# samson6460/tf2_YOLO

Hardware: AMD Instinct MI355X
Metric: images/sec training YOLOv3 416x416 bs=32/GPU (higher is better)
Workload: dtype f32-storage/fp16x2-mfma

## Files before the change

### include/yolo_hip.h

```cpp
#ifndef YOLO_HIP_H_
#define YOLO_HIP_H_

#include <stddef.h>
#include <stdint.h>

#ifdef __cplusplus
extern "C" {
#endif

typedef enum yolo_status {
  YOLO_OK = 0,
  YOLO_ERR_INVALID_ARG = -1,
  YOLO_ERR_LAUNCH = -2,
  YOLO_ERR_WORKSPACE = -3
} yolo_status;

enum { YOLO_ACT_LINEAR = 0, YOLO_ACT_LEAKY = 1, YOLO_ACT_MISH = 2 };
enum { YOLO_HEAD_V3 = 3, YOLO_HEAD_V2 = 2, YOLO_HEAD_V1 = 1, YOLO_HEAD_V4 = 4 };
enum { YOLO_NMS_HARD = 1, YOLO_NMS_SOFT = 2, YOLO_NMS_DIOU = 3 };

const char* yolo_last_error(void);
int yolo_abi_version(void);
int yolo_device_available(void);
int yolo_mfma_probe(const void* operands_f16, float* sink, int workgroups, int iters, double* flops_host, void* stream);

enum { YOLO_OPT_CONV_WIN = 0, YOLO_OPT_STAMPS = 1, YOLO_OPT_CONV_SK = 2, YOLO_OPT_CONV_PATCH = 5, YOLO_OPT_WGRAD_WIN = 6,
       YOLO_OPT_NMS_WALK = 7 ,
       YOLO_OPT_AB = 8  };
int yolo_set_option(int key, int value);
const char* yolo_last_conv_kernel(int* launches_host);
size_t yolo_conv_workspace_bytes(void);
int yolo_set_conv_workspace(void* p, size_t bytes, void* stream);
int yolo_set_debug_buffer(void* p, size_t bytes);

typedef struct yolo_conv_desc {
  int N, H, W, Cin;
  int Cout, kh, kw;
  int Ho, Wo;
  int sh, sw;
  int pad_t, pad_l;
} yolo_conv_desc;

#define YOLO_BN_STAT_SLOTS 64
#define YOLO_BN_RED_SLOTS 512
#define YOLO_SPLIT_BATCH_UNITS 4

int yolo_conv2d_fwd(const yolo_conv_desc* d, const float* x, const float* w,
                    const float* bias, float* y, double* stats, void* stream);
int yolo_conv2d_fwd_absmax(const yolo_conv_desc* d, const float* x, const float* w, const float* bias,
                           float* y, double* stats, unsigned* absmax, void* stream);

int yolo_conv2d_dgrad(const yolo_conv_desc* d, const float* dy, const float* wT,
                      float* dx, int accumulate, void* stream);

int yolo_conv2d_wgrad(const yolo_conv_desc* d, const float* x, const float* dy,
                      float* dw, float* dbias, void* stream);

int yolo_conv2d_wgrad_bias(const float* dy, long long P, int Cout, float* dbias, void* stream);

int yolo_filter_transpose(const float* w, float* wT, int Cout, int taps, int Cin, void* stream);

size_t yolo_planes_bytes(long long rows, int C);
// ... 303 lines not shown
```

### tf2_yolo_amd/_lib.py

```python
import ctypes
import os
from ctypes import (POINTER, Structure, c_char_p, c_double, c_float, c_int, c_longlong,
                    c_size_t, c_void_p)

from . import tape as _tape

_HERE = os.path.dirname(os.path.abspath(__file__))
LIB_PATH = os.path.join(_HERE, "libyolo_hip.so")

ACT_LINEAR, ACT_LEAKY, ACT_MISH = 0, 1, 2
PREC_F32, PREC_F16 = 0, 1
_PRECISIONS = {"fp32": PREC_F32, "fp16": PREC_F16}


def precision_enum(precision):
    try:
        return _PRECISIONS[precision]
    except (KeyError, TypeError):
        raise ValueError(f"precision must be 'fp32' or 'fp16', got {precision!r}") from None
NMS_HARD, NMS_SOFT, NMS_DIOU = 1, 2, 3


class YoloHipError(RuntimeError):
    pass


class ConvDesc(Structure):
    _fields_ = [(n, c_int) for n in
                ("N", "H", "W", "Cin", "Cout", "kh", "kw", "Ho", "Wo", "sh", "sw", "pad_t", "pad_l")]


class LossCfg(Structure):
    _fields_ = [("version", c_int), ("N", c_int), ("gh", c_int), ("gw", c_int), ("A", c_int),
                ("C", c_int), ("anchors", c_float * 32), ("use_anchors", c_int),
                ("binary_weight", c_float), ("loss_weight", c_float * 4),
                ("ignore_thresh", c_float), ("use_focal_loss", c_int), ("focal_gamma", c_float),
                ("use_scale", c_int), ("wh_reg_weight", c_float), ("truth_thresh", c_float),
                ("label_smooth", c_float)]


_P = c_void_p
_LL = c_longlong
SIGNATURES = {
    "yolo_last_error": (c_char_p, []),
    "yolo_abi_version": (c_int, []),
    "yolo_device_available": (c_int, []),
    "yolo_set_option": (c_int, [c_int, c_int]),
    "yolo_last_conv_kernel": (c_char_p, [POINTER(c_int)]),
    "yolo_mfma_probe": (c_int, [_P, _P, c_int, c_int, POINTER(c_double), _P]),
    "yolo_set_debug_buffer": (c_int, [_P, c_size_t]),
    "yolo_encode_labels": (c_int, [_P, _P, _P, c_int, c_double, c_double, c_int, c_int, c_int, _P, _P, _P]),
    "yolo_down2xlabel": (c_int, [_P, c_int, c_int, c_int, c_int, _P, _P, _P]),
    "yolo_conv_workspace_bytes": (c_size_t, []),
    "yolo_set_conv_workspace": (c_int, [_P, c_size_t, _P]),
    "yolo_conv2d_fwd": (c_int, [POINTER(ConvDesc), _P, _P, _P, _P, _P, _P]),
    "yolo_conv2d_dgrad": (c_int, [POINTER(ConvDesc), _P, _P, _P, c_int, _P]),
    "yolo_conv2d_wgrad": (c_int, [POINTER(ConvDesc), _P, _P, _P, _P, _P]),
    "yolo_conv2d_wgrad_bias": (c_int, [_P, _LL, c_int, _P, _P]),
    "yolo_filter_transpose": (c_int, [_P, _P, c_int, c_int, c_int, _P]),
    "yolo_planes_bytes": (c_size_t, [_LL, c_int]),
    "yolo_split_planes": (c_int, [_P, _LL, c_int, _P, _P]),
    "yolo_split_planes_padded": (c_int, [_P, _LL, c_int, c_int, _P, _P]),
    "yolo_split_planes_batch": (c_int, [_P, c_int, _LL, _P]),
    "yolo_filter_transpose_batch": (c_int, [_P, c_int, _LL, _P]),
    "yolo_conv2d_fwd_planes": (c_int, [POINTER(ConvDesc), _P, _P, _P, _P, _P, _P, _P]),
    "yolo_stem_bwd_scratch_bytes": (c_size_t, []),
    "yolo_stem_bn_bwd_wgrad": (c_int, [POINTER(ConvDesc), _P, _P, _P, _P, _P, _P, _P, c_int, _P, _P, _P, _P, _P, c_size_t, _P]),
    "yolo_conv2d_fwd_planes_epi": (c_int, [POINTER(ConvDesc), _P, _P, _P, c_int, _P, _P, _P, _P, _P, _P]),
    "yolo_split_planes_absmax": (c_int, [_P, _LL, c_int, _P, _P, _P, _P, _P]),
    "yolo_conv_pred_bound": (c_int, [_P, c_int, c_int, _P, _P, _P, _P, _P]),
    "yolo_conv2d_fwd_infer_unit": (c_int, [POINTER(ConvDesc), _P, _P, _P, c_int, _P, _P, _P, _P, _P, _P, _P, c_int, _P, c_int,
                                           _P, _P, _P, POINTER(c_int), _P]),
    "yolo_fold_bound": (c_int, [_P, c_int, _P, _P]),
    "yolo_absmax_words": (c_int, [_P, _LL, _P, POINTER(c_int), _P]),
    "yolo_stem_filter_prep": (c_int, [_P, _P, _P, _P]),
    "yolo_stem_fwd_infer_unit": (c_int, [POINTER(ConvDesc), _P, _P, c_int, _P, _P, _P, _P, c_int, _P, _P, _P, POINTER(c_int), _P]),
    "yolo_split_planes_concat": (c_int, [POINTER(c_void_p), POINTER(c_int), POINTER(c_void_p), c_int, _LL, _P, _P, _P, _P]),
    "yolo_split_planes_concat_ex": (c_int, [POINTER(c_void_p), POINTER(c_int), POINTER(c_void_p), POINTER(c_int), POINTER(c_int),
                                            c_int, c_int, c_int, _LL, _P, _P, _P, _P]),
    "yolo_conv2d_fwd_head_unit": (c_int, [POINTER(ConvDesc), _P, _P, _P, c_int, c_int, c_int, _P, _P, _P, _P]),
# ... 78 lines not shown
    "yolo_nms_workspace_bytes": (c_size_t, [c_int, c_int]),
    "yolo_cal_iou": (c_int, [_P, _P, _P, _P, c_int, c_int, c_int, POINTER(c_longlong), POINTER(c_longlong),
                             POINTER(c_longlong), c_double, c_double, _P]),
    "yolo_match_detections": (c_int, [_P, c_int, _P, c_int, c_int, c_double, _P, _P, _P, _P, _P, _P]),
    "yolo_rank_desc": (c_int, [_P, _P, c_int, _P, _P]),
    "yolo_pr_curve_workspace_bytes": (c_size_t, [c_int, c_int]),
    "yolo_pr_curve": (c_int, [_P, _P, _P, c_int, c_int, c_int, _P, c_size_t, _P, _P, _P]),
    "yolo_match_batch_workspace_bytes": (c_size_t, [c_int, c_int, c_int]),
    "yolo_match_batch": (c_int, [_P, c_int, _P, _P, c_int, _P, c_int, c_int, c_double, _P, _P, _P, _P, _P, _P, _P, c_size_t, _P]),
    "yolo_rank_desc_images": (c_int, [_P, _P, c_int, _P, c_int, _P, _P]),
    "yolo_pr_curves_workspace_bytes": (c_size_t, [c_int, c_int, _LL]),
    "yolo_pr_curves": (c_int, [_P, _P, _P, _P, c_int, _P, c_int, _LL, c_int, _P, c_size_t, _P, _P, _P, _P]),
    "yolo_nms": (c_int, [_P, c_int, c_int, c_int, c_double, c_double, c_double, _P, _P, c_size_t, _P]),
    "yolo_nms_select": (c_int, [_P, c_int, c_int, c_int, c_double, c_double, c_double, _P, _P, _P, _P, c_size_t, _P]),
    "yolo_decode_batch_workspace_bytes": (c_size_t, [c_int, POINTER(c_int), POINTER(c_int), POINTER(c_int), c_int, c_int]),
    "yolo_decode_batch_count": (c_int, [POINTER(c_void_p), POINTER(c_int), c_int, c_int, POINTER(c_int), POINTER(c_int),
                                        POINTER(c_int), c_int, c_int, POINTER(c_double), _P, _P, c_size_t, _P]),
    "yolo_decode_batch_write": (c_int, [POINTER(c_void_p), POINTER(c_int), c_int, c_int, POINTER(c_int), POINTER(c_int),
                                        POINTER(c_int), c_int, c_int, POINTER(c_double), _P, c_int, _P, c_size_t, _P]),
    "yolo_nms_batch_workspace_bytes": (c_size_t, [c_int, c_int, c_int]),
    "yolo_nms_batch_prepare": (c_int, [_P, c_int, _P, c_int, c_int, _P, _P, c_size_t, _P]),
    "yolo_nms_batch_select": (c_int, [_P, c_int, c_int, c_int, c_int, c_double, c_double, c_double, _P, _LL, _P, _P, _P, _P,
                                      c_size_t, _P]),
    "yolo_image_prepare": (c_int, [_P, _LL, _P, c_int, c_int, c_int, c_float, c_float, _P, _P]),
}

_lib = None

_QUERIES = {"yolo_last_error", "yolo_last_conv_kernel", "yolo_abi_version", "yolo_bnred_slots_cap", "yolo_device_available", "yolo_conv_workspace_bytes", "yolo_planes_bytes",
            "yolo_stem_bwd_scratch_bytes", "yolo_loss_workspace_bytes", "yolo_decode_workspace_bytes",
            "yolo_nms_workspace_bytes", "yolo_pr_curve_workspace_bytes", "yolo_wgrad_workspace_bytes", "yolo_adam_lr_t",
            "yolo_grad_sqnorm_workspace_bytes", "yolo_decode_batch_workspace_bytes", "yolo_nms_batch_workspace_bytes",
            "yolo_match_batch_workspace_bytes", "yolo_pr_curves_workspace_bytes",
            "yolo_set_option", "yolo_set_debug_buffer", "yolo_set_conv_workspace", "yolo_set_wgrad_workspace"}


class _Recorded:
    __slots__ = ("f", "name")

    def __init__(self, f, name):
        self.f, self.name = f, name

    def __call__(self, *a):
        rc = self.f(*a)
        if _tape.ACTIVE is not None:
            _tape.ACTIVE.c(self.f, a, self.name)
        return rc


class _Lib:

    def __init__(self, cdll):
        self._cdll = cdll

    def __getattr__(self, name):
        f = getattr(self._cdll, name)
        if name not in _QUERIES and name in SIGNATURES:
            f = _Recorded(f, name)
        setattr(self, name, f)
        return f


def load():
    global _lib
    if _lib is not None:
        return _lib
    if not os.path.exists(LIB_PATH):
# ... 24 lines not shown
```

### tf2_yolo_amd/csrc/conv_args.hpp

```cpp
#pragma once
#include "common.hpp"

namespace yolo {

constexpr int MAX_TAPS = 49;

struct Tap {
  int oy, ox, woff;
};

struct ClassGeom {
  long long M;
  int Hg, Wg, ooy, oox, tap0, ntaps;
};

struct GatherConvArgs {
  const float* src;
  const float* wgt;
  const float* bias;
  float* dst;
  double* stats;
  unsigned* absmax;
  long long M;
  int N, Hs, Ws, Cs;
// ... 68 lines not shown
  long long M;
  int N, Hs, Ws, Cs;
  int Hg, Wg;
  int sy, sx;
  int Cout, ldw;
  int ntaps;
  int kw, pad_t, pad_l;
  int tiles_co, tiles_j;
  int nblocks;
  long long chunk;
  unsigned src_bytes, dy_bytes;
  int zero_blk_src, zero_blk_dy;
  float* slabs;
  int splits;
};

int launch_gather_split(GatherConvArgs& a, hipStream_t st);
bool gather_split_supported(const GatherConvArgs& a);
long long planes_bytes(long long rows, int C);
int launch_split_planes(const float* x, long long rows, int C, void* planes, hipStream_t st);
int launch_split_planes_absmax(const float* x, long long rows, int C, const unsigned* absmax, const float* extra_bound, int extra_n,
                               void* planes, float* out_bound, hipStream_t st);
int launch_split_planes_concat(const float* const* xs, const int* Cs, const float* const* bounds, int nsrc, long long rows,
                               void* planes, float* dst32, float* out_bound, hipStream_t st,
                               const int* bound_words = nullptr, const int* upsample = nullptr, int H = 0, int W = 0);
int launch_split_planes_padded(const float* x, long long rows, int Csrc, int C, void* planes, hipStream_t st);
int launch_split_planes_batch(const void* jobs, int njobs, long long total_blocks, hipStream_t st);
int launch_filter_transpose_batch(const void* jobs, int njobs, long long total_blocks, hipStream_t st);
int launch_gather_planes(GatherConvArgs& a, hipStream_t st);
bool conv_small_supported(const GatherConvArgs& a);
bool conv_small_head_supported(const GatherConvArgs& a);
int launch_conv_small(GatherConvArgs& a, hipStream_t st, int* nwg);
bool gather_planes_supported(const GatherConvArgs& a);
int conv_split_parts(const GatherConvArgs& a, long long nb, int bm, int min_cb, int idle_div);
int launch_split_reduce(GatherConvArgs& a, int bm, hipStream_t st);
float* conv_split_slabs();
int launch_conv_win(GatherConvArgs& a, int variant, hipStream_t st);
bool conv_win_supported(const GatherConvArgs& a);
enum { OPT_CONV_WIN = 0, OPT_STAMPS = 1, OPT_CONV_SK = 2, OPT_DBG = 3, OPT_TILE_ORDER = 4, OPT_CONV_PATCH = 5, OPT_WGRAD_WIN = 6, OPT_NMS_WALK = 7, OPT_EXP = 8, OPT_COUNT = 16 };
int set_conv_workspace(void* p, size_t bytes, hipStream_t st);
extern void* g_dbg_buf;
extern size_t g_dbg_bytes;
extern int g_opt[OPT_COUNT];
void init_options();
void note_conv_launch(const char* family, int a = 0, int b = 0, int c = 0, int d = 0);
int launch_wgrad_planes(WgradArgs& a, hipStream_t st);
bool wgrad_planes_supported(const WgradArgs& a);
int launch_wgrad_win(WgradArgs& a, hipStream_t st);
bool wgrad_win_supported(const WgradArgs& a);
constexpr size_t WGRAD_WS_COLSUM_BYTES = 1 << 20;
void* wgrad_workspace(size_t* bytes);
bool stem_fwd_supported(const yolo_conv_desc* d);
struct StemEpiArgs {
  const float* scale;
  const float* shift;
  int act;
  void* planes;
  const float* pred;
  const unsigned* in_words;
  int in_n;
  unsigned* out_words;
};
bool stem_infer_supported(const yolo_conv_desc* d);
int launch_stem_filter_prep(const float* w, const float* bias, float* wt, hipStream_t st);
int launch_absmax_words(const float* x, long long n, unsigned* words, int* n_words, hipStream_t st);
int launch_stem_infer(const yolo_conv_desc* d, const float* x, const float* wt, float* y, const StemEpiArgs& e, int* out_n,
                      hipStream_t st);
size_t stem_bwd_scratch_bytes();
int launch_stem_bn_bwd_wgrad(const yolo_conv_desc* d, const float* y, const float* dout, const float* img, const float* scale,
                             const float* shift, const float* smean, const float* sinv, int act, const double* redsum,
                             float* dgamma, float* dbeta, float* dw, float* scratch, size_t scratch_bytes, hipStream_t st);
int launch_stem_fwd(const yolo_conv_desc* d, const float* x, const float* w, const float* bias, float* y, double* stats,
// ... 6 lines not shown
```

### tf2_yolo_amd/csrc/conv_planes.hip

```cpp
#include "planes_epilogue.hpp"
#include <algorithm>
#include <cstdlib>
#include <type_traits>

namespace yolo {

__global__ __launch_bounds__(256) void planes_amax_kernel(const float* __restrict__ x, long long n4,
                                                         unsigned* __restrict__ header) {
  float m = 0.f;
  for (long long i = (long long)blockIdx.x * 256 + threadIdx.x; i < n4; i += (long long)gridDim.x * 256) {
    const f32x4 v = reinterpret_cast<const f32x4*>(x)[i];
    m = fmaxf(fmaxf(m, fmaxf(fabsf(v[0]), fabsf(v[1]))), fmaxf(fabsf(v[2]), fabsf(v[3])));
  }
#pragma unroll
  for (int o = 32; o > 0; o >>= 1) m = fmaxf(m, __shfl_xor(m, o, 64));
  __shared__ float wmax[4];
  if ((threadIdx.x & 63) == 0) wmax[threadIdx.x >> 6] = m;
  __syncthreads();
  if (threadIdx.x == 0) {
    m = fmaxf(fmaxf(wmax[0], wmax[1]), fmaxf(wmax[2], wmax[3]));
    if (__builtin_bit_cast(unsigned, m) > *reinterpret_cast<volatile unsigned*>(header))
      atomicMax(header, __builtin_bit_cast(unsigned, m));
  }
}
// ... 198 lines not shown
                                                                 long long rows_padded) {
  unsigned* header = reinterpret_cast<unsigned*>(out + planes_body_bytes(rows, C));
  const float sc = planes_scale_from_bound(header[0]);
  const int G = C >> 3;
  const long long t = (long long)blockIdx.x * 256 + threadIdx.x;
  if (t == 0) {
    reinterpret_cast<float*>(header)[1] = sc;
    reinterpret_cast<float*>(header)[2] = 1.f / sc;
  }
  if (t >= rows_padded * G) return;
  const long long row = t / G;
  const int g = (int)(t - row * G);
  f32x4 v0 = {0.f, 0.f, 0.f, 0.f}, v1 = {0.f, 0.f, 0.f, 0.f};
  if (row < rows) {
    const float* p = x + row * Csrc;
#pragma unroll
    for (int j = 0; j < 4; ++j) {
      if (g * 8 + j < Csrc) v0[j] = p[g * 8 + j];
      if (g * 8 + 4 + j < Csrc) v1[j] = p[g * 8 + 4 + j];
    }
  }
  const Planes8 s = split8(v0, v1, sc);
  unsigned char* o = out + planes_unit_offset(row, g, C);
  *reinterpret_cast<u32x4*>(o) = s.h;
  *reinterpret_cast<u32x4*>(o + 512) = s.l;
}

constexpr int PF_KO_MASK = 31;
constexpr int PF_SPLIT = 32;
constexpr int PF_MULTI = 64;
constexpr int PF_DEEP1 = 128;
constexpr int PF_DEEP2 = 256;
constexpr int PF_BNRED = 512;
template <int BM, int BN, int WGM, int WGN, int FORM = 0, int PASSES = 3>
__global__ __launch_bounds__(64 * WGM * WGN, (WGM * WGN >= 4 ? 2 : 1)) void gather_conv_planes_kernel(const GatherConvArgs a) {
  static_assert(planes_passes_ok(PASSES), "1 or 3 MFMA passes");
  static_assert(PASSES == 3 || (FORM & (PF_MULTI | PF_BNRED)) == 0, "one pass: forward inference forms only");
  constexpr int NPL = planes_frag_planes<PASSES>;
  constexpr int NW = WGM * WGN;
  constexpr int TM = BM / WGM / 32;
  constexpr int TN = BN / WGN / 32;
  constexpr int RBA = BM / 32, RBB = BN / 32;
  constexpr int LPW = (RBA + RBB + NW - 1) / NW;
  static_assert(LPW <= 4, "loader layout: slot s = wave + i*NW loads A block s, or B block (s - RBA) % RBB");
  constexpr int ND = PL_PLANES * LPW;
  constexpr int STAGE_BYTES = (RBA + RBB) * PL_PLANES * 1024;
  constexpr int NBUF = 3 + ((FORM >> 7) & 3);

  extern __shared__ __attribute__((aligned(16))) unsigned char smem[];
  const unsigned lds_base = (unsigned)(size_t)smem;

  const int tid = threadIdx.x;
  const int lane = tid & 63;
  const int wave = __builtin_amdgcn_readfirstlane(tid >> 6);
  const int wm = wave / WGN, wn = wave % WGN;

  constexpr bool SPLIT = (FORM & PF_SPLIT) != 0;
  const int SP = SPLIT ? a.split_parts : 1;
  const int part = SPLIT ? (int)blockIdx.x / a.nblocks : 0;
  const int tile = xcd_remap(SPLIT ? (int)blockIdx.x - part * a.nblocks : (int)blockIdx.x, a.nblocks);
  constexpr bool MULTI = (FORM & PF_MULTI) != 0;
  constexpr bool BNRED = (FORM & PF_BNRED) != 0;
  const int tile_n = tile % a.tiles_n;
  const int cls = MULTI ? (tile / a.tiles_n) % a.ncls : 0;
  const int tile_m = MULTI ? tile / (a.tiles_n * a.ncls) : tile / a.tiles_n;
  const long long m0 = (long long)tile_m * BM;
  const int n0 = tile_n * BN;
  const EpiGeom G = MULTI ? EpiGeom{a.cls[cls].M, a.cls[cls].Hg, a.cls[cls].Wg, a.cls[cls].ooy, a.cls[cls].oox, 0, 0, 0,
                                    tile_m * a.ncls + cls + 1}
                          : epi_geom_of(a);
  const int tap0 = MULTI ? a.cls[cls].tap0 : 0;
  const int ntaps = MULTI ? a.cls[cls].ntaps : a.ntaps;
  if (MULTI && m0 >= G.M) {
    if (a.bwd_y != nullptr)
      for (int c = tid; c < BN; c += 64 * NW)
        if (n0 + c < a.Cout) {
          a.bwd_part[((long long)(G.slot1 - 1) * 2 + 0) * a.Cout + n0 + c] = 0.f;
          a.bwd_part[((long long)(G.slot1 - 1) * 2 + 1) * a.Cout + n0 + c] = 0.f;
        }
    return;
  }
  const int HgWg = G.Hg * G.Wg;

  const int r = lane & 31, hf = lane >> 5;
  const unsigned blkstrideA = (unsigned)((a.Cs >> 4) * PL_RECORD);
  const unsigned blkstrideB = (unsigned)((a.ldw >> 4) * PL_RECORD);
  const i32x4 rsrcA = planes_rsrc(a.src, a.src_bytes), rsrcB = planes_rsrc(a.wgt, a.wgt_bytes);
  const int cpt_all = a.Cs >> 4;
  const int cb_lo = (part * cpt_all) / SP;
  const int cpt = ((part + 1) * cpt_all) / SP;
  const int nk = ntaps * (cpt - cb_lo);

  bool isA[LPW];
  int nimg[LPW], ys0[LPW], xs0[LPW];
  unsigned rowbaseB[LPW], lds_mine[LPW], ld_voff[LPW], ld_soff[LPW];
#pragma unroll
  for (int i = 0; i < LPW; ++i) {
    const int slot = wave + i * NW;
    isA[i] = slot < RBA;
    const int rb = isA[i] ? slot : (slot - RBA) % RBB;
    nimg[i] = 0; ys0[i] = -(1 << 28); xs0[i] = 0; rowbaseB[i] = 0;
    if (isA[i]) {
      const long long m = m0 + rb * 32 + r;
      if (m < G.M) {
        nimg[i] = (int)(m / HgWg);
        const int rem = (int)(m - (long long)nimg[i] * HgWg);
        const int y = rem / G.Wg;
        ys0[i] = y * a.sy;
        xs0[i] = (rem - y * G.Wg) * a.sx;
      }
    } else {
      const int co = n0 + rb * 32 + r;
      const unsigned blk = co < a.Cout ? (unsigned)(co >> 4) : (unsigned)a.zero_blk_wgt;
      rowbaseB[i] = blk * blkstrideB + (co < a.Cout ? (co & 15) * 16 : 0) + hf * 256;
    }
    lds_mine[i] = lds_base + ((isA[i] ? 0 : RBA) + rb) * PL_PLANES * 1024;
    ld_voff[i] = 0; ld_soff[i] = 0;
  }

  int ld_tap = 0, ld_kk = 0, ld_cb = cb_lo;
  auto loader_tap = [&]() {
#pragma unroll
    for (int i = 0; i < LPW; ++i) {
      if (ld_cb >= cpt) {
        ld_voff[i] = isA[i] ? (unsigned)a.zero_blk_src * blkstrideA : (unsigned)a.zero_blk_wgt * blkstrideB;
        ld_soff[i] = 0;
      } else if (isA[i]) {
        const int ys = ys0[i] + a.taps[tap0 + ld_tap].oy, xs = xs0[i] + a.taps[tap0 + ld_tap].ox;
        const bool ok = ((unsigned)ys < (unsigned)a.Hs) && ((unsigned)xs < (unsigned)a.Ws);
        const int pix = (nimg[i] * a.Hs + ys) * a.Ws + xs;
        ld_voff[i] = (ok ? ((unsigned)pix >> 4) : (unsigned)a.zero_blk_src) * blkstrideA + (ok ? (pix & 15) * 16 : 0) + hf * 256;
        ld_soff[i] = (unsigned)ld_cb * PL_RECORD;
      } else {
        ld_voff[i] = rowbaseB[i];
        ld_soff[i] = (unsigned)((a.taps[tap0 + ld_tap].woff >> 4) + ld_cb) * PL_RECORD;
      }
    }
// ... 78 lines not shown
  loader_tap();
#pragma unroll
  for (int b = 0; b < NBUF; ++b) issue_stage(b);
  asm volatile("s_waitcnt vmcnt(%0)" ::"n"((NBUF - 1) * ND) : "memory");
  __builtin_amdgcn_s_barrier();
  read_frags(0, S0{});

  auto step = [&](int rbuf, int wbuf, auto CUR, auto NXT) {
    asm volatile("s_waitcnt vmcnt(%0)" ::"n"((NBUF - 2) * ND) : "memory");
    asm volatile("s_waitcnt lgkmcnt(0)" ::: "memory");
    if constexpr (!(FORM & 4)) __builtin_amdgcn_s_barrier();
    if constexpr (!(FORM & 2)) read_frags(rbuf, NXT);
    __builtin_amdgcn_sched_barrier(0);
    mfma_stage(CUR, wbuf);
  };
  {
    int rbuf = 1, wbuf = 0;
    int kt = 0;
    for (; kt + 1 < nk; kt += 2) {
      step(rbuf, wbuf, S0{}, S1{});
      rbuf = (rbuf + 1 == NBUF) ? 0 : rbuf + 1;
      wbuf = (wbuf + 1 == NBUF) ? 0 : wbuf + 1;
      step(rbuf, wbuf, S1{}, S0{});
      rbuf = (rbuf + 1 == NBUF) ? 0 : rbuf + 1;
      wbuf = (wbuf + 1 == NBUF) ? 0 : wbuf + 1;
    }
    if (kt < nk) step(rbuf, wbuf, S0{}, S1{});
  }
  asm volatile("s_waitcnt vmcnt(0)" ::: "memory");
  __syncthreads();

  if constexpr (SPLIT)
    store_split_slab<TM, TN>(a, acc, BM * BN * 4, tile * SP + part, wave, lane);
  else if constexpr (MULTI)
    planes_epilogue<BM, BN, WGM, WGN, NBUF * STAGE_BYTES, 0, NoStamp, false, BNRED>(a, acc, smem, m0, n0, tile_m, wm, wn, lane, tid, NoStamp(), &G);
  else
    planes_epilogue<BM, BN, WGM, WGN, NBUF * STAGE_BYTES, (FORM & PF_KO_MASK), NoStamp, false, BNRED>(a, acc, smem, m0, n0, tile_m, wm, wn, lane, tid);
}

template <int BM, int BN, int WGM, int WGN, int FORM = 0>
static int launch_planes(GatherConvArgs& a, hipStream_t st) {
  const long long tiles_m = (a.M + BM - 1) / BM;
  a.tiles_n = (a.Cout + BN - 1) / BN;
  const long long nb = tiles_m * a.tiles_n;
  if (nb <= 0 || nb > 0x7fffffffLL) {
    set_error("conv(planes): bad grid %lld", nb);
    return YOLO_ERR_INVALID_ARG;
  }
  note_conv_launch("gather_conv_planes_kernel<%d,%d,%d,%d>", BM, BN, WGM, WGN);
  constexpr size_t lds = (3 + ((FORM >> 7) & 3)) * (BM / 32 + BN / 32) * PL_PLANES * 1024;
  const dim3 block(64 * WGM * WGN);
  if constexpr (FORM == 0) {
    if (a.ncls > 1) {
      long long tm = 0;
      for (int c = 0; c < a.ncls; ++c) tm = std::max(tm, (a.cls[c].M + BM - 1) / BM);
      const long long nbm = tm * a.ncls * a.tiles_n;
      if (nbm <= 0 || nbm > 0x7fffffffLL) {
        set_error("conv(planes): bad grid %lld", nbm);
        return YOLO_ERR_INVALID_ARG;
      }
      a.nblocks = (int)nbm;
      a.split_parts = 1;
      a.bwd_nslots = (int)(tm * a.ncls);
      YOLO_BNRED_CHECK(a)
      if (a.bwd_y == nullptr)
        return launch_lds<gather_conv_planes_kernel<BM, BN, WGM, WGN, PF_MULTI>, lds>(dim3((unsigned)nbm), block, st, a,
                                                                                      "gather_conv_planes_kernel(classes)");
      return launch_lds<gather_conv_planes_kernel<BM, BN, WGM, WGN, PF_MULTI | PF_BNRED>, lds>(
          dim3((unsigned)nbm), block, st, a, "gather_conv_planes_kernel(classes, bn reduce)");
    }
  }
  a.nblocks = (int)nb;
  a.bwd_nslots = (int)tiles_m;
  YOLO_BNRED_CHECK(a)
  constexpr auto plain = &gather_conv_planes_kernel<BM, BN, WGM, WGN, FORM>;
  constexpr bool HAS_ONE_PASS = (FORM & ~(PF_DEEP1 | PF_DEEP2)) == 0;
  if (a.one_pass && (!HAS_ONE_PASS || a.stats != nullptr || a.bwd_y != nullptr || a.accumulate)) {
    set_error("conv(planes): one MFMA pass is an inference-forward form only");
    return YOLO_ERR_INVALID_ARG;
  }
  a.split_parts = 1;
  if constexpr (BM == 128 && BN == 128 && WGM == 2 && WGN == 2 && FORM == 0) {
    const int min_cb = a.ntaps >= 8 ? 1 : (8 + a.ntaps - 1) / a.ntaps;
    a.split_parts = conv_split_parts(a, nb, BM, min_cb, 4);
    if (a.split_parts > 1) {
      a.sk_slabs = conv_split_slabs();
      const int rc = a.one_pass ? launch_lds<gather_conv_planes_kernel<BM, BN, WGM, WGN, PF_SPLIT, 1>, lds>(
                                      dim3((unsigned)(nb * a.split_parts)), block, st, a, "gather_conv_planes_kernel(split, one pass)")
                                : launch_lds<gather_conv_planes_kernel<BM, BN, WGM, WGN, PF_SPLIT>, lds>(
                                      dim3((unsigned)(nb * a.split_parts)), block, st, a, "gather_conv_planes_kernel(split)");
      if (rc) return rc;
      return launch_split_reduce(a, BM, st);
    }
  }
  if constexpr ((FORM & ~(PF_DEEP1 | PF_DEEP2)) == 0) {
    if (a.bwd_y != nullptr)
      return launch_lds<gather_conv_planes_kernel<BM, BN, WGM, WGN, FORM | PF_BNRED>, lds>(dim3((unsigned)nb), block, st, a,
                                                                                          "gather_conv_planes_kernel(bn reduce)");
  } else if (a.bwd_y != nullptr) {
    set_error("conv(planes): this diagnostic instantiation has no fused BatchNorm-backward reduction");
    return YOLO_ERR_INVALID_ARG;
  }
  if constexpr (HAS_ONE_PASS) {
    if (a.one_pass)
      return launch_lds<gather_conv_planes_kernel<BM, BN, WGM, WGN, FORM, 1>, lds>(dim3((unsigned)nb), block, st, a,
                                                                                  "gather_conv_planes_kernel(one pass)");
  }
  return launch_lds<plain, lds>(dim3((unsigned)nb), block, st, a, "gather_conv_planes_kernel");
}

long long planes_bytes(long long rows, int C) { return planes_body_bytes(rows, C) + PL_HEADER; }

bool gather_planes_supported(const GatherConvArgs& a) { return (a.Cs % 16) == 0 && a.Cout >= 32; }

int launch_gather_planes(GatherConvArgs& a, hipStream_t st) {
  const long long rowsA = (long long)a.N * a.Hs * a.Ws;
  const long long bytesA = planes_bytes(rowsA, a.Cs), bytesB = planes_bytes(a.Cout, a.ldw);
  if (bytesA >= (1LL << 32) || bytesB >= (1LL << 32)) {
    set_error("conv(planes): operand planes exceed 4 GiB (%lld, %lld bytes)", bytesA, bytesB);
    return YOLO_ERR_INVALID_ARG;
  }
  a.src_bytes = (unsigned)bytesA;
  a.wgt_bytes = (unsigned)bytesB;
  a.zero_blk_src = (int)((rowsA + 15) / 16);
  a.zero_blk_wgt = (a.Cout + 15) / 16;
  static const int nt = env_int("YOLO_NT_STORE", 1);
  a.nt_store = nt;
  static const int vecst = env_int("YOLO_VEC_STORE", 1);
  a.vec_store = vecst;
  static const int dbg = env_int("YOLO_PLANES_DBG", 0);
  a.dbg = dbg;
  static const int kc_env = env_int("YOLO_PLANES_KC", 0);
  a.kc = kc_env > 0 ? kc_env : (a.Cs >> 4);
  if (a.kc > (a.Cs >> 4)) a.kc = a.Cs >> 4;
  init_options();
  if (g_opt[OPT_CONV_WIN] != 0 && a.ncls <= 1) {
    const int rc = launch_conv_win(a, g_opt[OPT_CONV_WIN], st);
    if (rc <= 0) return rc;
  }
  static const int deep_env = env_int("YOLO_PLANES_DEEP", -1);
  const int deep = deep_env >= 0 ? deep_env : (a.Cout <= 64 ? 1 : 2);
  if (deep && a.ntaps == 1 && a.ncls <= 1) {
    if (a.Cout <= 32) return deep == 1 ? launch_planes<128, 32, 4, 1, PF_DEEP1>(a, st) : launch_planes<128, 32, 4, 1, PF_DEEP2>(a, st);
    if (a.Cout <= 64) return deep == 1 ? launch_planes<128, 64, 4, 2, PF_DEEP1>(a, st) : launch_planes<128, 64, 4, 2, PF_DEEP2>(a, st);
  }
  if (a.Cout <= 32) return launch_planes<128, 32, 4, 1>(a, st);
  if (a.Cout <= 64) return launch_planes<128, 64, 4, 2>(a, st);
  static const int narrow_below = env_int("YOLO_PLANES_NARROW_BELOW", 0);
  if (((a.M + 127) / 128) * ((a.Cout + 127) / 128) < narrow_below) return launch_planes<128, 64, 4, 2>(a, st);
  static const int waves_env = env_int("YOLO_PLANES_WAVES", 0);
  const int waves = waves_env ? waves_env : (a.ntaps == 1 && a.ncls <= 1 ? 8 : 4);
#ifdef YOLO_PLANES_KNOCKOUTS
  switch (a.dbg) {
    case 1: return launch_planes<128, 128, 2, 2, 1>(a, st);
    case 2: return launch_planes<128, 128, 2, 2, 2>(a, st);
    case 3: return launch_planes<128, 128, 2, 2, 3>(a, st);
    case 7: return launch_planes<128, 128, 2, 2, 7>(a, st);
    case 8: return launch_planes<128, 128, 2, 2, 8>(a, st);
    case 11: return launch_planes<128, 128, 2, 2, 11>(a, st);
    case 15: return launch_planes<128, 128, 2, 2, 15>(a, st);
    case 16: return launch_planes<128, 128, 2, 2, 16>(a, st);
    case 23: return launch_planes<128, 128, 2, 2, 23>(a, st);
    case 31: return launch_planes<128, 128, 2, 2, 31>(a, st);
    default: break;
  }
#endif
  if (waves == 2) return launch_planes<128, 128, 2, 1>(a, st);
  if (waves == 4) {
// ... 266 lines not shown
```

### tf2_yolo_amd/csrc/planes_epilogue.hpp

```cpp
#pragma once
#include "planes.hpp"
#include "act.hpp"

namespace yolo {

struct NoStamp {
  __device__ __forceinline__ void operator()(int) const {}
};

struct EpiGeom {
  long long M;
  int Hg, Wg, ooy, oox;
  int pn, py0, px0;
  int slot1;
};
__device__ __forceinline__ EpiGeom epi_geom_of(const GatherConvArgs& a) {
  return EpiGeom{a.M, a.Hg, a.Wg, a.ooy, a.oox, 0, 0, 0, 0};
}

template <int TM, int TN>
__device__ __forceinline__ void store_split_slab(const GatherConvArgs& a, f32x16 (&acc)[TM][TN], const int slab_bytes,
                                                 const int slab, const int wave, const int lane) {
  unsigned char* mine = reinterpret_cast<unsigned char*>(a.sk_slabs) + (size_t)slab * slab_bytes;
  const __amdgpu_buffer_rsrc_t rs = __builtin_amdgcn_make_buffer_rsrc(mine, 0, slab_bytes, 0x00020000);
#pragma unroll
  for (int i = 0; i < TM; ++i)
#pragma unroll
    for (int j = 0; j < TN; ++j)
#pragma unroll
      for (int q4 = 0; q4 < 4; ++q4) {
        const f32x4 f = {acc[i][j][4 * q4], acc[i][j][4 * q4 + 1], acc[i][j][4 * q4 + 2], acc[i][j][4 * q4 + 3]};
        __builtin_amdgcn_raw_buffer_store_b128(__builtin_bit_cast(u32x4, f), rs,
                                               (((wave * TM + i) * TN + j) * 4 + q4) * 1024 + lane * 16, 0, 0);
      }
}

template <int BM, int BN, int WGM, int WGN, int LDS_BYTES, int DBG = 0, class STAMP = NoStamp, bool PATCH = false, bool BNRED = false>
__device__ __forceinline__ void planes_epilogue(const GatherConvArgs& a, f32x16 (&acc)[BM / WGM / 32][BN / WGN / 32],
                                                unsigned char* smem, const long long m0, const int n0, const int tile_m,
                                                const int wm, const int wn, const int lane, const int tid,
                                                const STAMP& stampf = STAMP(), const EpiGeom* geom = nullptr) {
  const EpiGeom G = geom != nullptr ? *geom : epi_geom_of(a);
  constexpr int NT = 64 * WGM * WGN;
  constexpr int NW = WGM * WGN;
  constexpr int TM = BM / WGM / 32;
  constexpr int TN = BN / WGN / 32;
  const int wave = wm * WGN + wn;
  float* smf = reinterpret_cast<float*>(smem);
  long long* rowoff = reinterpret_cast<long long*>(smf);
  const bool dense = a.osy == 1 && a.osx == 1 && G.ooy == 0 && G.oox == 0 && a.Hd == G.Hg && a.Wd == G.Wg;
  {
    const int HgWg = G.Hg * G.Wg;
    for (int rr = tid; rr < BM; rr += NT) {
      const long long m = m0 + rr;
      long long off = -1;
      if constexpr (PATCH) {
        const int y = G.py0 + (rr >> 4), x = G.px0 + (rr & 15);
        if (y < G.Hg && x < G.Wg) off = (((long long)G.pn * a.Hd + y) * a.Wd + x) * a.Cd;
      } else if (m < G.M) {
        if (dense) {
          off = m * a.Cd;
        } else {
          const int n = (int)(m / HgWg);
          const int rem = (int)(m - (long long)n * HgWg);
          const int y = rem / G.Wg;
          const int x = rem - y * G.Wg;
          off = (((long long)n * a.Hd + (y * a.osy + G.ooy)) * a.Wd + (x * a.osx + G.oox)) * a.Cd;
        }
      }
      rowoff[rr] = off;
    }
  }
  __syncthreads();
  stampf(0);

  const float unscale =
      reinterpret_cast<const float*>(reinterpret_cast<const unsigned char*>(a.src) + a.src_bytes - PL_HEADER)[2] *
      reinterpret_cast<const float*>(reinterpret_cast<const unsigned char*>(a.wgt) + a.wgt_bytes - PL_HEADER)[2];
  float* sred = smf + 2 * BM;
  float csum[TN], csq[TN], cmx[TN];
#pragma unroll
  for (int j = 0; j < TN; ++j) csum[j] = csq[j] = cmx[j] = 0.f;
  [[maybe_unused]] float bs1[TN], bs2[TN];
#pragma unroll
  for (int j = 0; j < TN; ++j) bs1[j] = bs2[j] = 0.f;
  asm volatile("" ::"v"(unscale));
  stampf(1);
  const int rows_valid = PATCH ? BM : ((G.M - m0 < (long long)BM) ? (int)(G.M - m0) : BM);
  const bool want_stats = a.stats != nullptr || a.absmax != nullptr;
  [[maybe_unused]] unsigned long long rowmask = ~0ull;
  if constexpr (PATCH) {
// ... 304 lines not shown
```

### tf2_yolo_amd/csrc/runtime.hip

```cpp
#include "conv_args.hpp"
#include <cstdlib>
#include <cstring>

namespace yolo {

static thread_local char g_err[512] = "";

void set_error(const char* fmt, ...) {
  va_list ap;
  va_start(ap, fmt);
  vsnprintf(g_err, sizeof(g_err), fmt, ap);
  va_end(ap);
}

static thread_local struct { const char* family; int v[4]; int launches; } g_conv_note = {"", {0, 0, 0, 0}, 0};
static thread_local char g_conv_name[96] = "";

void note_conv_launch(const char* family, int a, int b, int c, int d) {
  g_conv_note = {family, {a, b, c, d}, g_conv_note.launches + 1};
}

int g_opt[OPT_COUNT];
void* g_dbg_buf = nullptr;
size_t g_dbg_bytes = 0;
static void options_from_env() {
  for (int i = 0; i < OPT_COUNT; ++i) g_opt[i] = 0;
  g_opt[OPT_CONV_WIN] = env_int("YOLO_CONV_WIN", 1);
  g_opt[OPT_CONV_SK] = env_int("YOLO_CONV_SK", 1);
  g_opt[OPT_CONV_PATCH] = env_int("YOLO_CONV_PATCH", 1);
  g_opt[OPT_WGRAD_WIN] = env_int("YOLO_WGRAD_WIN", 1);
  g_opt[OPT_NMS_WALK] = env_int("YOLO_NMS_WALK", 0);
  g_opt[OPT_EXP] = env_int("YOLO_EXP", 0);
}
void init_options() {
  static bool done = false;
  if (done) return;
  done = true;
  options_from_env();
}

}

extern "C" int yolo_set_option(int key, int value) {
  yolo::init_options();
  if (key == -1) {
    yolo::options_from_env();
    return YOLO_OK;
  }
  if (key < 0 || key >= yolo::OPT_COUNT) {
    yolo::set_error("yolo_set_option: unknown key %d", key);
    return YOLO_ERR_INVALID_ARG;
  }
  yolo::g_opt[key] = value;
  return YOLO_OK;
}

extern "C" size_t yolo_conv_workspace_bytes(void) { return (size_t)(1 << 20) + (size_t)512 * 2 * 256 * 128 * 4; }

extern "C" int yolo_set_conv_workspace(void* p, size_t bytes, void* stream) {
  yolo::init_options();
  return yolo::set_conv_workspace(p, bytes, yolo::as_stream(stream));
}

extern "C" int yolo_set_debug_buffer(void* p, size_t bytes) {
  yolo::g_dbg_buf = p;
  yolo::g_dbg_bytes = bytes;
  return YOLO_OK;
}

extern "C" const char* yolo_last_error(void) { return yolo::g_err; }

extern "C" const char* yolo_last_conv_kernel(int* launches) {
  auto& n = yolo::g_conv_note;
  snprintf(yolo::g_conv_name, sizeof(yolo::g_conv_name), n.family, n.v[0], n.v[1], n.v[2], n.v[3]);
  if (launches != nullptr) *launches = n.launches;
  n = {"", {0, 0, 0, 0}, 0};
  return yolo::g_conv_name;
}

extern "C" int yolo_abi_version(void) { return 5; }

#include <dlfcn.h>
namespace {
using nccl_allreduce_fn = int (*)(const void*, void*, size_t, int, int, void*, hipStream_t);
nccl_allreduce_fn find_nccl_allreduce() {
  void* f = dlsym(RTLD_DEFAULT, "ncclAllReduce");
  if (f == nullptr) {
// ... 30 lines not shown
```

### tf2_yolo_amd/ops.py

```python
import ctypes
from ctypes import byref, c_void_p

import torch

from . import _lib
from . import tape as _tape
from ._lib import ConvDesc, LossCfg, YoloHipError, check

BN_EPS = 1e-3
BN_MOMENTUM = 0.99
BN_STAT_SLOTS = 64
BN_RED_SLOTS = 512
SPLIT_BATCH_UNITS = 4


class KernelTimer:

    def __init__(self):
        self.pending = []

    def bracket(self, flops, fn, layer=None):
        last, n = _lib.load().yolo_last_conv_kernel, ctypes.c_int(0)
        last(None)
        s, e = torch.cuda.Event(enable_timing=True), torch.cuda.Event(enable_timing=True)
# ... 20 lines not shown
TIMER = None


def _conv_flops(d):
    return 2.0 * d.N * d.Ho * d.Wo * d.Cout * d.kh * d.kw * d.Cin


def _layer_key(d, which):
    return (which, d.H, d.W, d.Cin, d.Cout, d.kh, d.sh, d.N)


import os as _os
CONV_MODE = "fp32" if _os.environ.get("YOLO_CONV_MODE", "split")[:1] in ("f", "0") else "split"
USE_PLANES = CONV_MODE == "split" and _os.environ.get("YOLO_CONV_PLANES", "1") != "0"


def planes_fwd_ok(cin, cout):
    return USE_PLANES and cin % 16 == 0 and cout >= 32


def planes_dgrad_ok(cin, cout):
    return USE_PLANES and cout % 16 == 0 and cin >= 32


def planes_wgrad_ok(cin, cout, taps, stride=1):
    return USE_PLANES and cin % 16 == 0 and cout % 16 == 0 and cout >= 32 and taps * cin >= 64


OPT_CONV_WIN = 0
OPT_CONV_SK = 2
OPT_CONV_PATCH = 5
OPT_WGRAD_WIN = 6
OPT_NMS_WALK = 7
_CONV_WS = None


def ensure_conv_workspace():
    global _CONV_WS
    if _CONV_WS is not None and _CONV_WS.device.index != torch.cuda.current_device():
        raise YoloHipError(f"libyolo_hip.so was initialised on cuda:{_CONV_WS.device.index} and cannot also serve "
                           f"cuda:{torch.cuda.current_device()}: start one process per GPU")
    if _CONV_WS is None:
        lib = _lib.load()
        n = int(lib.yolo_conv_workspace_bytes())
        _CONV_WS = torch.empty(n, dtype=torch.uint8, device="cuda")
        check(lib.yolo_set_conv_workspace(_p(_CONV_WS), n, _stream()), "yolo_set_conv_workspace")
    return _CONV_WS


_WGRAD_WS = None


def ensure_wgrad_workspace():
    global _WGRAD_WS
    if _WGRAD_WS is None:
        lib = _lib.load()
        n = int(lib.yolo_wgrad_workspace_bytes())
        _WGRAD_WS = torch.empty(n, dtype=torch.uint8, device="cuda")
        check(lib.yolo_set_wgrad_workspace(_p(_WGRAD_WS), n), "yolo_set_wgrad_workspace")
    return _WGRAD_WS


_SIDE_STREAMS = {}


def _overlaps(a, b, cycles=6000000):
    e0, e1, e2 = (torch.cuda.Event(enable_timing=True) for _ in range(3))
# ... 1331 lines not shown
```

Measured before the change: 1085.

## Add 2D patch tiling for planes conv and adaptive K-chunk policy

Adds an optional kernel form that maps each 128-row tile to an 8x16 spatial patch of one image instead of a linear pixel range. The aim is better input reuse across overlapping taps. It also adds a default-on policy that shrinks the per-pass channel chunk (kc) for multi-tap convolutions with many tiles, targeting about 32 tap-chunks per pass. The patch path is off by default and uses padded tiles at the image edges. The chunk policy changes pipeline granularity for all eligible layers.

```diff
diff --git a/include/yolo_hip.h b/include/yolo_hip.h
--- a/include/yolo_hip.h
+++ b/include/yolo_hip.h
@@ -26,8 +26,10 @@
 
 enum { YOLO_OPT_CONV_WIN = 0, YOLO_OPT_STAMPS = 1, YOLO_OPT_CONV_SK = 2, YOLO_OPT_CONV_PATCH = 5, YOLO_OPT_WGRAD_WIN = 6,
        YOLO_OPT_NMS_WALK = 7 ,
-       YOLO_OPT_AB = 8  };
+       YOLO_OPT_AB = 8 ,
+       YOLO_OPT_PLANES_PATCH = 9, YOLO_OPT_PLANES_CHUNK = 10 };
 int yolo_set_option(int key, int value);
+int yolo_planes_patch_policy(int mode, int ntaps, int N, int Hg, int Wg, int Cout);
 const char* yolo_last_conv_kernel(int* launches_host);
 size_t yolo_conv_workspace_bytes(void);
 int yolo_set_conv_workspace(void* p, size_t bytes, void* stream);
diff --git a/tf2_yolo_amd/_lib.py b/tf2_yolo_amd/_lib.py
--- a/tf2_yolo_amd/_lib.py
+++ b/tf2_yolo_amd/_lib.py
@@ -46,6 +46,7 @@
     "yolo_abi_version": (c_int, []),
     "yolo_device_available": (c_int, []),
     "yolo_set_option": (c_int, [c_int, c_int]),
+    "yolo_planes_patch_policy": (c_int, [c_int, c_int, c_int, c_int, c_int, c_int]),
     "yolo_last_conv_kernel": (c_char_p, [POINTER(c_int)]),
     "yolo_mfma_probe": (c_int, [_P, _P, c_int, c_int, POINTER(c_double), _P]),
     "yolo_set_debug_buffer": (c_int, [_P, c_size_t]),
@@ -190,7 +191,7 @@
             "yolo_nms_workspace_bytes", "yolo_pr_curve_workspace_bytes", "yolo_wgrad_workspace_bytes", "yolo_adam_lr_t",
             "yolo_grad_sqnorm_workspace_bytes", "yolo_decode_batch_workspace_bytes", "yolo_nms_batch_workspace_bytes",
             "yolo_match_batch_workspace_bytes", "yolo_pr_curves_workspace_bytes",
-            "yolo_set_option", "yolo_set_debug_buffer", "yolo_set_conv_workspace", "yolo_set_wgrad_workspace"}
+            "yolo_planes_patch_policy", "yolo_set_option", "yolo_set_debug_buffer", "yolo_set_conv_workspace", "yolo_set_wgrad_workspace"}
 
 
 class _Recorded:
diff --git a/tf2_yolo_amd/csrc/conv_args.hpp b/tf2_yolo_amd/csrc/conv_args.hpp
--- a/tf2_yolo_amd/csrc/conv_args.hpp
+++ b/tf2_yolo_amd/csrc/conv_args.hpp
@@ -124,12 +124,15 @@
 bool conv_small_head_supported(const GatherConvArgs& a);
 int launch_conv_small(GatherConvArgs& a, hipStream_t st, int* nwg);
 bool gather_planes_supported(const GatherConvArgs& a);
+bool planes_patch_policy(int mode, int ntaps, int N, int Hg, int Wg, int Cout);
+int planes_chunk_policy(int mode, int ntaps, int ncls, long long tiles, int cpt);
 int conv_split_parts(const GatherConvArgs& a, long long nb, int bm, int min_cb, int idle_div);
 int launch_split_reduce(GatherConvArgs& a, int bm, hipStream_t st);
 float* conv_split_slabs();
 int launch_conv_win(GatherConvArgs& a, int variant, hipStream_t st);
 bool conv_win_supported(const GatherConvArgs& a);
-enum { OPT_CONV_WIN = 0, OPT_STAMPS = 1, OPT_CONV_SK = 2, OPT_DBG = 3, OPT_TILE_ORDER = 4, OPT_CONV_PATCH = 5, OPT_WGRAD_WIN = 6, OPT_NMS_WALK = 7, OPT_EXP = 8, OPT_COUNT = 16 };
+enum { OPT_CONV_WIN = 0, OPT_STAMPS = 1, OPT_CONV_SK = 2, OPT_DBG = 3, OPT_TILE_ORDER = 4, OPT_CONV_PATCH = 5, OPT_WGRAD_WIN = 6, OPT_NMS_WALK = 7, OPT_EXP = 8,
+       OPT_PLANES_PATCH = 9, OPT_PLANES_CHUNK = 10, OPT_COUNT = 16 };
 int set_conv_workspace(void* p, size_t bytes, hipStream_t st);
 extern void* g_dbg_buf;
 extern size_t g_dbg_bytes;
diff --git a/tf2_yolo_amd/csrc/conv_planes.hip b/tf2_yolo_amd/csrc/conv_planes.hip
--- a/tf2_yolo_amd/csrc/conv_planes.hip
+++ b/tf2_yolo_amd/csrc/conv_planes.hip
@@ -254,6 +254,7 @@
 constexpr int PF_DEEP1 = 128;
 constexpr int PF_DEEP2 = 256;
 constexpr int PF_BNRED = 512;
+constexpr int PF_PATCH = 1024;
 template <int BM, int BN, int WGM, int WGN, int FORM = 0, int PASSES = 3>
 __global__ __launch_bounds__(64 * WGM * WGN, (WGM * WGN >= 4 ? 2 : 1)) void gather_conv_planes_kernel(const GatherConvArgs a) {
   static_assert(planes_passes_ok(PASSES), "1 or 3 MFMA passes");
@@ -283,17 +284,29 @@
   const int tile = xcd_remap(SPLIT ? (int)blockIdx.x - part * a.nblocks : (int)blockIdx.x, a.nblocks);
   constexpr bool MULTI = (FORM & PF_MULTI) != 0;
   constexpr bool BNRED = (FORM & PF_BNRED) != 0;
+  constexpr bool PATCH = (FORM & PF_PATCH) != 0;
+  static_assert(!PATCH || (BM == 128 && (FORM & (PF_SPLIT | PF_BNRED | PF_DEEP1 | PF_DEEP2)) == 0 && PASSES == 3),
+                "patch tiles: 8 x 16 pixels, plain and multi-class three-pass forms only");
   const int tile_n = tile % a.tiles_n;
   const int cls = MULTI ? (tile / a.tiles_n) % a.ncls : 0;
   const int tile_m = MULTI ? tile / (a.tiles_n * a.ncls) : tile / a.tiles_n;
   const long long m0 = (long long)tile_m * BM;
   const int n0 = tile_n * BN;
-  const EpiGeom G = MULTI ? EpiGeom{a.cls[cls].M, a.cls[cls].Hg, a.cls[cls].Wg, a.cls[cls].ooy, a.cls[cls].oox, 0, 0, 0,
-                                    tile_m * a.ncls + cls + 1}
-                          : epi_geom_of(a);
+  EpiGeom G = MULTI ? EpiGeom{a.cls[cls].M, a.cls[cls].Hg, a.cls[cls].Wg, a.cls[cls].ooy, a.cls[cls].oox, 0, 0, 0,
+                              tile_m * a.ncls + cls + 1}
+                    : epi_geom_of(a);
   const int tap0 = MULTI ? a.cls[cls].tap0 : 0;
   const int ntaps = MULTI ? a.cls[cls].ntaps : a.ntaps;
-  if (MULTI && m0 >= G.M) {
+  bool past_end = m0 >= G.M;
+  if constexpr (PATCH) {
+    const int tx = (G.Wg + 15) >> 4, ty = (G.Hg + 7) >> 3;
+    G.pn = tile_m / (tx * ty);
+    const int rem = tile_m - G.pn * (tx * ty);
+    G.py0 = (rem / tx) * 8;
+    G.px0 = (rem % tx) * 16;
+    past_end = G.pn >= a.N;
+  }
+  if (MULTI && past_end) {
     if (a.bwd_y != nullptr)
       for (int c = tid; c < BN; c += 64 * NW)
         if (n0 + c < a.Cout) {
@@ -324,7 +337,14 @@
     nimg[i] = 0; ys0[i] = -(1 << 28); xs0[i] = 0; rowbaseB[i] = 0;
     if (isA[i]) {
       const long long m = m0 + rb * 32 + r;
-      if (m < G.M) {
+      if constexpr (PATCH) {
+        const int y = G.py0 + ((rb * 32 + r) >> 4), x = G.px0 + (r & 15);
+        if (y < G.Hg && x < G.Wg) {
+          nimg[i] = G.pn;
+          ys0[i] = y * a.sy;
+          xs0[i] = x * a.sx;
+        }
+      } else if (m < G.M) {
         nimg[i] = (int)(m / HgWg);
         const int rem = (int)(m - (long long)nimg[i] * HgWg);
         const int y = rem / G.Wg;
@@ -469,16 +489,42 @@
 
   if constexpr (SPLIT)
     store_split_slab<TM, TN>(a, acc, BM * BN * 4, tile * SP + part, wave, lane);
-  else if constexpr (MULTI)
-    planes_epilogue<BM, BN, WGM, WGN, NBUF * STAGE_BYTES, 0, NoStamp, false, BNRED>(a, acc, smem, m0, n0, tile_m, wm, wn, lane, tid, NoStamp(), &G);
+  else if constexpr (MULTI || PATCH)
+    planes_epilogue<BM, BN, WGM, WGN, NBUF * STAGE_BYTES, 0, NoStamp, PATCH, BNRED>(a, acc, smem, m0, n0, tile_m, wm, wn, lane, tid, NoStamp(), &G);
   else
     planes_epilogue<BM, BN, WGM, WGN, NBUF * STAGE_BYTES, (FORM & PF_KO_MASK), NoStamp, false, BNRED>(a, acc, smem, m0, n0, tile_m, wm, wn, lane, tid);
+}
+
+bool planes_patch_policy(int mode, int ntaps, int N, int Hg, int Wg, int Cout) {
+  if (mode == 0 || N <= 0 || Hg <= 0 || Wg <= 0 || Cout <= 0) return false;
+  if (mode != 1) return true;
+  const int bn = Cout <= 32 ? 32 : Cout <= 64 ? 64 : 128;
+  const long long ty = (Hg + 7) / 8, tx = (Wg + 15) / 16;
+  const long long tiles = (long long)N * ty * tx * ((Cout + bn - 1) / bn);
+  return ntaps > 1 && tiles >= 256 && 100 * (ty * 8) * (tx * 16) <= 108LL * Hg * Wg;
+}
+int planes_chunk_policy(int mode, int ntaps, int ncls, long long tiles, int cpt) {
+  if (mode <= 0 || ntaps <= 1 || cpt <= 1) return cpt;
+  if (mode >= 2) return mode - 1 < cpt ? mode - 1 : cpt;
+  if (ncls > 1 || tiles < 256) return cpt;
+  const int want = 32 / ntaps > 1 ? 32 / ntaps : 1;
+  const int nch = (cpt + want - 1) / want;
+  return (cpt + nch - 1) / nch;
 }
 
 template <int BM, int BN, int WGM, int WGN, int FORM = 0>
 static int launch_planes(GatherConvArgs& a, hipStream_t st) {
   const long long tiles_m = (a.M + BM - 1) / BM;
   a.tiles_n = (a.Cout + BN - 1) / BN;
+  constexpr bool HAS_PATCH = FORM == 0 && BM == 128 && ((BN == 32 && WGM == 4 && WGN == 1) || (BN == 64 && WGM == 4 && WGN == 2) ||
+                                                        (BN == 128 && WGM == 2 && WGN == 2));
+  [[maybe_unused]] bool patch = false;
+  if constexpr (HAS_PATCH) {
+    int nt = a.ntaps;
+    for (int c = 0; c < a.ncls; ++c) nt = std::max(nt, a.cls[c].ntaps);
+    patch = a.bwd_y == nullptr && !a.one_pass && planes_patch_policy(g_opt[OPT_PLANES_PATCH], nt, a.N, a.Hg, a.Wg, a.Cout);
+  }
+  auto patches = [&](int Hg, int Wg) { return (long long)a.N * ((Hg + 7) / 8) * ((Wg + 15) / 16); };
   const long long nb = tiles_m * a.tiles_n;
   if (nb <= 0 || nb > 0x7fffffffLL) {
     set_error("conv(planes): bad grid %lld", nb);
@@ -490,7 +536,7 @@
   if constexpr (FORM == 0) {
     if (a.ncls > 1) {
       long long tm = 0;
-      for (int c = 0; c < a.ncls; ++c) tm = std::max(tm, (a.cls[c].M + BM - 1) / BM);
+      for (int c = 0; c < a.ncls; ++c) tm = std::max(tm, patch ? patches(a.cls[c].Hg, a.cls[c].Wg) : (a.cls[c].M + BM - 1) / BM);
       const long long nbm = tm * a.ncls * a.tiles_n;
       if (nbm <= 0 || nbm > 0x7fffffffLL) {
         set_error("conv(planes): bad grid %lld", nbm);
@@ -500,6 +546,11 @@
       a.split_parts = 1;
       a.bwd_nslots = (int)(tm * a.ncls);
       YOLO_BNRED_CHECK(a)
+      if constexpr (HAS_PATCH) {
+        if (patch)
+          return launch_lds<gather_conv_planes_kernel<BM, BN, WGM, WGN, PF_MULTI | PF_PATCH>, lds>(
+              dim3((unsigned)nbm), block, st, a, "gather_conv_planes_kernel(classes, patch)");
+      }
       if (a.bwd_y == nullptr)
         return launch_lds<gather_conv_planes_kernel<BM, BN, WGM, WGN, PF_MULTI>, lds>(dim3((unsigned)nbm), block, st, a,
                                                                                       "gather_conv_planes_kernel(classes)");
@@ -543,6 +594,18 @@
       return launch_lds<gather_conv_planes_kernel<BM, BN, WGM, WGN, FORM, 1>, lds>(dim3((unsigned)nb), block, st, a,
                                                                                   "gather_conv_planes_kernel(one pass)");
   }
+  if constexpr (HAS_PATCH) {
+    if (patch) {
+      const long long nbp = patches(a.Hg, a.Wg) * a.tiles_n;
+      if (nbp > 0x7fffffffLL) {
+        set_error("conv(planes): bad grid %lld", nbp);
+        return YOLO_ERR_INVALID_ARG;
+      }
+      a.nblocks = (int)nbp;
+      return launch_lds<gather_conv_planes_kernel<BM, BN, WGM, WGN, PF_PATCH>, lds>(dim3((unsigned)nbp), block, st, a,
+                                                                                   "gather_conv_planes_kernel(patch)");
+    }
+  }
   return launch_lds<plain, lds>(dim3((unsigned)nb), block, st, a, "gather_conv_planes_kernel");
 }
 
@@ -567,10 +630,16 @@
   a.vec_store = vecst;
   static const int dbg = env_int("YOLO_PLANES_DBG", 0);
   a.dbg = dbg;
+  init_options();
   static const int kc_env = env_int("YOLO_PLANES_KC", 0);
-  a.kc = kc_env > 0 ? kc_env : (a.Cs >> 4);
+  {
+    int nt = a.ntaps;
+    for (int c = 0; c < a.ncls; ++c) nt = std::max(nt, a.cls[c].ntaps);
+    const int bn = a.Cout <= 32 ? 32 : a.Cout <= 64 ? 64 : 128;
+    const long long tiles = ((a.M + 127) / 128) * ((a.Cout + bn - 1) / bn) * (a.ncls > 1 ? a.ncls : 1);
+    a.kc = kc_env > 0 ? kc_env : planes_chunk_policy(a.one_pass ? 0 : g_opt[OPT_PLANES_CHUNK], nt, a.ncls, tiles, a.Cs >> 4);
+  }
   if (a.kc > (a.Cs >> 4)) a.kc = a.Cs >> 4;
-  init_options();
   if (g_opt[OPT_CONV_WIN] != 0 && a.ncls <= 1) {
     const int rc = launch_conv_win(a, g_opt[OPT_CONV_WIN], st);
     if (rc <= 0) return rc;
diff --git a/tf2_yolo_amd/csrc/planes_epilogue.hpp b/tf2_yolo_amd/csrc/planes_epilogue.hpp
--- a/tf2_yolo_amd/csrc/planes_epilogue.hpp
+++ b/tf2_yolo_amd/csrc/planes_epilogue.hpp
@@ -56,7 +56,8 @@
       long long off = -1;
       if constexpr (PATCH) {
         const int y = G.py0 + (rr >> 4), x = G.px0 + (rr & 15);
-        if (y < G.Hg && x < G.Wg) off = (((long long)G.pn * a.Hd + y) * a.Wd + x) * a.Cd;
+        if (y < G.Hg && x < G.Wg)
+          off = (((long long)G.pn * a.Hd + (y * a.osy + G.ooy)) * a.Wd + (x * a.osx + G.oox)) * a.Cd;
       } else if (m < G.M) {
         if (dense) {
           off = m * a.Cd;
diff --git a/tf2_yolo_amd/csrc/runtime.hip b/tf2_yolo_amd/csrc/runtime.hip
--- a/tf2_yolo_amd/csrc/runtime.hip
+++ b/tf2_yolo_amd/csrc/runtime.hip
@@ -31,6 +31,8 @@
   g_opt[OPT_WGRAD_WIN] = env_int("YOLO_WGRAD_WIN", 1);
   g_opt[OPT_NMS_WALK] = env_int("YOLO_NMS_WALK", 0);
   g_opt[OPT_EXP] = env_int("YOLO_EXP", 0);
+  g_opt[OPT_PLANES_PATCH] = env_int("YOLO_PLANES_PATCH", 0);
+  g_opt[OPT_PLANES_CHUNK] = env_int("YOLO_PLANES_CHUNK", 1);
 }
 void init_options() {
   static bool done = false;
@@ -53,6 +55,10 @@
   }
   yolo::g_opt[key] = value;
   return YOLO_OK;
+}
+
+extern "C" int yolo_planes_patch_policy(int mode, int ntaps, int N, int Hg, int Wg, int Cout) {
+  return yolo::planes_patch_policy(mode, ntaps, N, Hg, Wg, Cout) ? 1 : 0;
 }
 
 extern "C" size_t yolo_conv_workspace_bytes(void) { return (size_t)(1 << 20) + (size_t)512 * 2 * 256 * 128 * 4; }
diff --git a/tf2_yolo_amd/ops.py b/tf2_yolo_amd/ops.py
--- a/tf2_yolo_amd/ops.py
+++ b/tf2_yolo_amd/ops.py
@@ -76,7 +76,13 @@
 OPT_CONV_PATCH = 5
 OPT_WGRAD_WIN = 6
 OPT_NMS_WALK = 7
+OPT_PLANES_PATCH = 9
+OPT_PLANES_CHUNK = 10
 _CONV_WS = None
+
+
+def planes_patch_policy(mode, ntaps, n, hg, wg, cout):
+    return bool(_lib.load().yolo_planes_patch_policy(int(mode), int(ntaps), int(n), int(hg), int(wg), int(cout)))
 
 
 def ensure_conv_workspace():
```

Measured after the change: 1086, median of 2. About the same (+0.0%).
